# kije/HSLU_I.BA_RAYTRACING.F2501_raytracer

Measured on AMD Instinct MI355X. Metric: Mray/s (primary+secondary, rays counted as the reference casts them), semesterbild@high_resolution, higher is better.
Workload: dtype f32; 1 GPU; semesterbild@high_resolution+anti_aliasing+soft_shadows (text.obj); width=1620, height=1350, rays_per_frame=34992000, rays_traced_per_frame=19683000, pixels_written=1768966, objects=14578, lights=50, parallelism=tiles48x48/1gpu, frames_in_flight=2, build_id=962c7787e075b4de-p0s0w0o6, queue_bytes=0, scene_budget_bytes=2147483648, phases=0

## Files before the change

### hslu_i/ba_raytracing/f2501_raytracer_amd/csrc/rt_api.cpp

```cpp
#include <hip/hip_runtime.h>

#include <algorithm>
#include <chrono>
#include <cmath>
#include <cstdio>
#include <cstdlib>
#include <cstring>
#include <string>
#include <vector>

#include "rt_cell_resolve.h"
#include "rt_host.h"

static void trace_point(hipStream_t stream, const char* what, uint32_t a = 0, uint32_t b = 0, uint32_t c = 0);
#define RC_TRY(expr) do { const int rc_ = (expr); if (rc_ != RT_OK) return rc_; } while (0)

extern "C" {

#ifndef RT_BUILD_ID
#define RT_BUILD_ID "unknown"
#endif
const char* rt_build_id(void) { return RT_BUILD_ID; }

int rt_selftest_exact_math(int device, const float* in, float* out_sqrt, float* out_rcp, uint32_t n) {
  if (!in || !out_sqrt || !out_rcp) return fail(RT_ERR_INVALID_ARG, "null argument");
  if (device < 0 || device >= rt_device_count()) return fail(RT_ERR_INVALID_ARG, "device %d out of range", device);
  HIP_TRY(hipSetDevice(device));
  DevBuf b;
  int rc = b.ensure((size_t)n * 12 + 12);
  if (rc != RT_OK) return rc;
  float* d = (float*)b.p;
  HIP_TRY(hipMemcpy(d, in, (size_t)n * 4, hipMemcpyHostToDevice));
  hipError_t e = (hipError_t)rt_launch_selftest_math(d, d + n, d + 2 * (size_t)n, n, nullptr);
  if (e != hipSuccess) {
    b.release();
    return fail(RT_ERR_HIP, "selftest launch failed: %s", hipGetErrorString(e));
  }
  hipError_t e1 = hipMemcpy(out_sqrt, d + n, (size_t)n * 4, hipMemcpyDeviceToHost);
  hipError_t e2 = hipMemcpy(out_rcp, d + 2 * (size_t)n, (size_t)n * 4, hipMemcpyDeviceToHost);
  b.release();
  if (e1 != hipSuccess || e2 != hipSuccess) return fail(RT_ERR_HIP, "selftest copy failed");
  return RT_OK;
}

// ... 220 lines not shown
    s->cloud_ball_f[0] = p->fw, s->cloud_ball_f[1] = p->fh, s->cloud_ball_f[2] = p->fd;
    rt_scale_cloud(s->cloud_host.data(), n, s->cloud_ball_f, &s->cloud_scaled, s->cloud_ball);
    HIP_TRY(hipMemcpyAsync(s->cloud.p, s->cloud_scaled.data(), n / 3 * 16, hipMemcpyHostToDevice, up.stream));
  }
  P->cloud_sets = (const float4*)s->cloud.p;
  memcpy(P->cloud_centre, s->cloud_ball, 12);
  P->cloud_delta = s->cloud_ball[3];
  rt_beam_constants(p->eps_distance, P);
  const uint32_t cap = p->tuning.shadow_candidate_cap;
  P->cand_cap = cap == RT_CAND_CAP_NONE ? 0u : (cap ? cap : 64u);
  return RT_OK;
}

static int prepare_receiver_flags(rt_scene* s, const rt_params* p, TableUpload& up, RtDevParams* P) {
  hipStream_t stream = up.stream;
  P->recv_flags = nullptr;
  if (p->tuning.no_receiver_flags || P->cand_cap == 0u) s->notes |= RT_NOTE_RECV_FLAGS_OFF_TUNING;
  if (!s->n_cells || !(P->cloud_delta > 0.0f)) s->notes |= RT_NOTE_RECV_FLAGS_OFF_SCENE;
  if (s->dev.n_lights > 8u) s->notes |= RT_NOTE_RECV_FLAGS_OFF_LIGHTS;
  if (p->traversal != RT_TRAVERSAL_BVH) s->notes |= RT_NOTE_RECV_FLAGS_OFF_TRAVERSAL;
  if (p->flags & RT_FLAG_BACKFACE_CULLING) s->notes |= RT_NOTE_RECV_FLAGS_OFF_CULLING;
  if (!p->tuning.no_receiver_flags && P->cand_cap != 0u && s->n_cells && s->dev.n_lights <= 8u && p->traversal == RT_TRAVERSAL_BVH &&
      !(p->flags & RT_FLAG_BACKFACE_CULLING) && P->cloud_delta > 0.0f) {
    const float key[8] = {P->beam_delta, p->eps_distance, P->cloud_centre[0], P->cloud_centre[1], P->cloud_centre[2], 1.f, 0.f, 0.f};
    if (memcmp(key, s->flags_key, sizeof(key)) != 0) {
      RC_TRY(up.begin());
      RtDevParams B = *P;
      B.flag_out = (uint16_t*)s->flags.p;
      B.flag_geo = (const float4*)s->flag_geo.p;
      B.n_cells = s->n_cells;
      B.n_tri_cells = s->n_tri_cells;
      s->cell_lists_built = false;
      s->cell_wide_built = false;
      B.cell_list_out = nullptr;
      const size_t list_bytes = (size_t)s->n_cells * s->dev.n_lights * 16u;
      size_t free_b = 0, total_b = 0;
      const size_t flag_bytes = s->flags.cap + s->flag_geo.cap;
      if (s->dev.n_slots <= 65533u && flag_bytes + list_bytes <= s->budget && hipMemGetInfo(&free_b, &total_b) == hipSuccess &&
          list_bytes <= (free_b + s->cell_lists.cap) / 4 && s->cell_lists.ensure(list_bytes + 64) == RT_OK) {
        HIP_TRY(hipMemsetAsync(s->cell_lists.p, 0xFF, list_bytes, stream));
        B.cell_list_out = (uint16_t*)s->cell_lists.p;
        s->cell_lists_built = true;
      }
      if (!s->cell_lists_built) s->cell_lists.release();
      hipError_t e = (hipError_t)rt_launch_flags(s->dev, B, stream);
      if (e != hipSuccess) return fail(RT_ERR_HIP, "rt_flags_kernel launch failed: %s", hipGetErrorString(e));
      trace_point(stream, "rt_flags_kernel: cells, lights, lists", s->n_cells, s->dev.n_lights, s->cell_lists_built ? 1u : 0u);
      static const char* const prune_env = getenv("RT_CELL_PRUNE");
      static const bool prune_off = prune_env && *prune_env == '0';
      if (s->cell_lists_built && !prune_off) {
        RtCellPruneArgs a{};
        a.flag_geo = (const float*)s->flag_geo.p;
        a.lists = (uint16_t*)s->cell_lists.p;
        a.flags = (uint16_t*)s->flags.p;
        a.n_cells = s->n_cells, a.n_tri_cells = s->n_tri_cells;
        memcpy(a.cloud_centre, P->cloud_centre, 12);
        a.beam_delta = P->beam_delta, a.beam_eps_o = P->beam_eps_o;
        a.mode = RT_PRUNE_FULL;
        e = (hipError_t)rt_launch_cell_prune(s->dev, a, stream);
        if (e != hipSuccess) return fail(RT_ERR_HIP, "rt_cell_prune_kernel launch failed: %s", hipGetErrorString(e));
        trace_point(stream, "rt_cell_prune_kernel: cells, lights", s->n_cells, s->dev.n_lights, 0u);
        static const char* const resolve_env = getenv("RT_CELL_RESOLVE");
        static const bool resolve_off = resolve_env && *resolve_env == '0';
        RtCellResolveArgs r{};
        const size_t temp_bytes = resolve_off ? 0 : rt_cell_resolve_temp_bytes(s->n_cells, s->budget - flag_bytes - list_bytes, &r.chunk_cells);
        if (temp_bytes && s->resolve_work.ensure(temp_bytes) == RT_OK) {
          r.cell = a;
          r.eps_push = P->beam_eps_push, r.eps_ulp = P->beam_eps_ulp;
          r.work = (uint32_t*)s->resolve_work.p;
          static const char* const wide_env = getenv("RT_CELL_WIDE");
          static const bool wide_off = wide_env && *wide_env == '0';
          const size_t used = flag_bytes + list_bytes + temp_bytes;
          const size_t wide_bytes = wide_off || used >= s->budget ? 0 : rt_cell_wide_pool_bytes(s->n_cells, s->dev.n_lights, s->budget - used, &r.wide_cap);
          if (wide_bytes && hipMemGetInfo(&free_b, &total_b) == hipSuccess && wide_bytes <= (free_b + s->cell_wide.cap) / 4 &&
              s->cell_wide.ensure(wide_bytes) == RT_OK) {
            r.wide = (uint16_t*)s->cell_wide.p;
            r.wide_count = (uint32_t*)((char*)s->cell_wide.p + (size_t)r.wide_cap * 2u * RT_CELL_WIDE_SLOTS);
            s->cell_wide_built = true;
          } else {
            r.wide_cap = 0u;
          }
          e = (hipError_t)rt_launch_cell_resolve(s->dev, r, stream);
          if (e != hipSuccess) return fail(RT_ERR_HIP, "rt_cell_resolve_kernel launch failed: %s", hipGetErrorString(e));
          trace_point(stream, "rt_cell_resolve_kernel: cells, lights, cells per chunk", s->n_cells, s->dev.n_lights, r.chunk_cells);
        } else {
          s->resolve_work.release();
        }
      }
      if (!s->cell_lists_built) s->resolve_work.release();
      if (!s->cell_wide_built) s->cell_wide.release();
      memcpy(s->flags_key, key, sizeof(key));
    }
    P->recv_flags = (const uint16_t*)s->flags.p;
    if (s->cell_lists_built && !p->tuning.no_cell_lists) P->cell_lists = (const uint4*)s->cell_lists.p;
    if (P->cell_lists && s->cell_wide_built) P->cell_wide = (const uint32_t*)s->cell_wide.p;
  }
  if (!P->cell_lists) s->notes |= RT_NOTE_CELL_LISTS_OFF;
  return RT_OK;
}

static void copy_frame_shape(rt_scene* s, const rt_params* p, uint32_t* argb_dev, const rt_aux* aux_dev, RtDevParams* P) {
  P->max_depth_reflection = p->max_depth_reflection;
  P->max_depth_refraction = p->max_depth_refraction;
  s->sort_bits_wanted = p->tuning.sort_bits;
  s->lanes_wanted = p->tuning.sub_frames;
  s->phases_wanted = p->tuning.phases;
  s->levels_wanted = p->tuning.levels;
  if (p->win_w) {
    P->win_x0 = p->win_x0, P->win_y0 = p->win_y0, P->win_w = p->win_w, P->win_h = p->win_h;
  } else {
    P->win_x0 = P->win_y0 = 0;
    P->win_w = p->width;
    P->win_h = p->height;
  }
  P->tile_size = p->tile_size ? p->tile_size : 48u;
  P->n_ranks = p->n_ranks;
  P->rank = p->rank;
  P->traversal = p->traversal;
  P->argb = argb_dev;
  if (aux_dev) {
    P->aux_rgb = aux_dev->rgb;
    P->aux_hit_id = aux_dev->hit_id;
    P->aux_hit_t = aux_dev->hit_t;
  }
}

static int take_frame_slot(rt_scene* s, const rt_params* p, hipStream_t stream, RtDevParams* P) {
  int blk = -1, oldest = 0, same = -1;
// ... 767 lines not shown
```

### hslu_i/ba_raytracing/f2501_raytracer_amd/csrc/rt_host.h

```cpp
#pragma once

#include <hip/hip_runtime.h>

#include <string>
#include <vector>

#include "rt_closest.h"
#include "rt_multihit.h"
#include "rt_ray_key.h"
#include "rt_scene_pack.h"

#define fail rt_fail

#define HIP_TRY(expr)                                                                          \
  do {                                                                                         \
    hipError_t e_ = (expr);                                                                    \
    if (e_ != hipSuccess)                                                                      \
      return fail(e_ == hipErrorOutOfMemory ? RT_ERR_OOM : RT_ERR_HIP, "%s failed: %s", #expr, \
                  hipGetErrorString(e_));                                                      \
  } while (0)

#define RT_SLOTS 4
#define RT_LANES 2
#define RT_MAX_DEPTH 64u
// ... 221 lines not shown
  std::vector<uint32_t> sup_host;
  uint32_t sup_key[8] = {0, 0, 0, 0, 0, 0, 0, 0};
  DevBuf costmap;
  std::vector<uint32_t> cost_host;
  uint32_t cost_key[13] = {0, 0, 0, 0, 0, 0, 0, 0, 0, 0, 0, 0, 0};
  bool cost_valid = false, cost_wanted = false;
  uint32_t q_cap = 0, hard_cap = 0, batch_items = 0;
  StreamKey stream_key{};
  uint32_t key_gen = 0;
  uint32_t sticky_notes = 0;
  bool stream_verified = false;
  uint32_t est[RT_LANES][RT_CNT_STRIDE] = {{0}};
  bool est_valid = false;
  uint32_t sort_bits_wanted = 0;
  uint32_t lanes_wanted = 0;
  uint32_t phases_wanted = 0;
  uint32_t levels_wanted = 0;
  uint32_t calm_frames = 1u << 30;
  uint32_t tables_version = 0;
  float aabb_lo[3] = {0.f, 0.f, 0.f}, aabb_hi[3] = {1.f, 1.f, 1.f};
  std::vector<float> aa_host, cloud_host, cloud_scaled;
  std::vector<uint32_t> aa_table;
  uint32_t aa_unique = 0;
  bool aa_dedup = true;
  hipEvent_t tables_ev = nullptr;
  hipStream_t tables_stream = nullptr, last_stream = nullptr;
  bool tables_pending = false, rendered = false;
  float cloud_ball[4] = {0.f, 0.f, 0.f, -1.f};
  DevBuf flag_geo, flags;
  DevBuf cell_lists;
  DevBuf resolve_work;
  DevBuf cell_wide;
  bool cell_wide_built = false;
  bool cell_lists_built = false;
  uint32_t n_cells = 0, n_tri_cells = 0;
  float flags_key[8] = {-1.f, 0.f, 0.f, 0.f, 0.f, 0.f, 0.f, 0.f};
  float cloud_ball_f[3] = {0.f, 0.f, 0.f};
  hipEvent_t frame_ev[RT_SLOTS] = {};
  bool frame_pending[RT_SLOTS] = {};
  uint32_t frame_seq[RT_SLOTS] = {};
  hipStream_t frame_stream[RT_SLOTS] = {};
  uint32_t frame_no = 0;
  int cur_block = 0, last_block = 0;
  int cur_ws = 0;
  int ws_last_block[RT_SLOTS] = {0, 1, 2, 3};
  uint32_t notes = 0;
  size_t queue_bytes = 0;
  RtRefitPlan plan;
  DevBuf plan_dev, upd_dev;
  size_t plan_off[5] = {0, 0, 0, 0, 0};
  void* upd_stage = nullptr;
  size_t upd_stage_cap = 0;
  float* upd_back = nullptr;
  uint64_t sah_created[2] = {0, 0};
  float sah_tri_cost = 2.0f;
  DevBuf sah_dev;
  uint32_t max_leaf = 4;
};


int rt_scene_upload_plan(rt_scene* s, const RtPackedScene& pk);
void rt_scene_release_update(rt_scene* s);

int rt_scene_wait_frames(rt_scene* s);

struct RtRebuildIn {
// ... 30 lines not shown
```

### hslu_i/ba_raytracing/f2501_raytracer_amd/csrc/rt_kernels.hip

```cpp
#include <hip/hip_runtime.h>

#include <stdlib.h>

#include <type_traits>

#include "rt_internal.h"

#define RT_EPS 1.1920929e-7f

#define RT_OPAQUE(v) asm volatile("" : "+v"(v))
#define RT_OPAQUE_S(v) asm volatile("" : "+s"(v))
typedef const __attribute__((address_space(4))) char* rt_kernarg_ptr;
__device__ __forceinline__ rt_kernarg_ptr kernarg_fresh() {
  rt_kernarg_ptr p = (rt_kernarg_ptr)__builtin_amdgcn_kernarg_segment_ptr();
  asm volatile("" : "+s"(p));
  return p;
}
#define RT_KERNARG_OFF_P ((sizeof(RtDevScene) + alignof(RtDevParams) - 1) / alignof(RtDevParams) * alignof(RtDevParams))
static_assert(RT_KERNARG_OFF_P == 88, "RtDevParams follows RtDevScene at kernarg offset 88");
__device__ __forceinline__ const RtDevScene& kernarg_scene() { return *(const RtDevScene*)(const char*)kernarg_fresh(); }
__device__ __forceinline__ const RtDevParams& kernarg_params() {
  return *(const RtDevParams*)((const char*)kernarg_fresh() + RT_KERNARG_OFF_P);
}
#define wave_ballot(pred) __builtin_amdgcn_ballot_w64((bool)(pred))
// ... 447 lines not shown
      if (CULL) h &= wave_ballot(dot(d, n) < 0.75f);
      S.occ |= h;
      return;
    }
    const OccConst k = occluder_constants(m);
    M.row = row;
    M.k.ar = uniform_u(k.ar), M.k.ag = uniform_u(k.ag), M.k.ab = uniform_u(k.ab), M.k.x = uniform_u(k.x);
    M.k.eta2_out = uniform_f(k.eta2_out), M.k.eta2_in = uniform_f(k.eta2_in), M.k.f0x = uniform_f(k.f0x);
    WSTAT(n_miss++);
  }
  WSTAT(n_exec++);
  shadow_add(S, M.k, n, d, h);
}

template <bool CULL>
__device__ __forceinline__ lanemask shadow_accumulate_lane(Shadow& S, const Mat& m, V3 n, V3 d, lanemask h) {
  if (CULL) h &= wave_ballot(m.transmissive || dot(d, n) < 0.75f);
  S.occ |= h & wave_ballot(!m.transmissive);
  const float io = m.transmissive ? m.opacity * (1.0f - fresnel_reflectance_air_red(m, n, -d)) : 0.0f;
  const bool on = lane_of(h);
  const uint32_t di = (uint32_t)__float2uint_rn(clampf(1.0f - io, 0.0f, 1.0f) * RT_SH_SCALE);
  const uint32_t nd = min(S.dec + di, RT_SH_ONE);
  S.dec = on ? nd : S.dec;
  const V3 ab = absorption(m);
  S.fr = on ? S.fr + (uint32_t)__float2uint_rn(ab.x * RT_FILT_SCALE) : S.fr;
  S.fg = on ? S.fg + (uint32_t)__float2uint_rn(ab.y * RT_FILT_SCALE) : S.fg;
  S.fb = on ? S.fb + (uint32_t)__float2uint_rn(ab.z * RT_FILT_SCALE) : S.fb;
  return h;
}

struct WaveCtx {
  uint32_t n_nodes, n_tris, s_nodes, s_tris, s_passes, n_exact, s_exact;
  uint32_t o_exec, o_miss;
#if RT_PROFILE
  unsigned long long t_mark;
  unsigned long long prof[7];
#endif
};

enum { CFG_TABLES_RUNTIME = -1, CFG_TABLES_FLAGS = 1, CFG_TABLES_LISTS = 2 };
struct CfgGeneric {
  static constexpr uint32_t N = 0u;
  static constexpr bool BVH = false;
  static constexpr int TABLES = CFG_TABLES_RUNTIME;
  static constexpr bool POW2_SETS = false;
  static constexpr bool FEW_SPHERES = false;
  static constexpr bool FAR_ORIGINS = false;
  static constexpr bool OCC_MEMO = false;
  static constexpr bool WIDE = false;
};
template <uint32_t N_, int TABLES_>
struct CfgSoft {
  static constexpr uint32_t N = N_;
  static constexpr bool BVH = true;
  static constexpr int TABLES = TABLES_;
  static constexpr bool POW2_SETS = true;
  static constexpr bool FEW_SPHERES = true;
  static constexpr bool FAR_ORIGINS = false;
  static constexpr bool OCC_MEMO = TABLES_ == CFG_TABLES_LISTS;
  static constexpr bool WIDE = TABLES_ == CFG_TABLES_LISTS;
};
struct CfgRays : CfgGeneric {
  static constexpr bool FAR_ORIGINS = true;
};

template <bool CULL, class C = CfgGeneric>
__device__ __forceinline__ Hit nearest_hit(const RtDevScene& sc, const RtDevParams& P, WaveCtx& W,
                                           bool alive, V3 o, V3 d) {
  Hit best;
  best.t = INFINITY;
  best.id = -1;
  const lanemask grp = wave_ballot(alive);
  uint32_t pre = 0xFFFFFFFFu;
  if (sc.n_spheres > 2u && grp) {
    const uint32_t ns = C::FEW_SPHERES ? sc.n_spheres : (sc.n_spheres < 32u ? sc.n_spheres : 32u);
    const int fl = __ffsll((long long)grp) - 1;
    auto first = [&](float v) { return __uint_as_float((uint32_t)__builtin_amdgcn_readlane((int)__float_as_uint(v), fl)); };
    const V3 o0 = mk(first(o.x), first(o.y), first(o.z)), d0 = mk(first(d.x), first(d.y), first(d.z));
    const V3 eo = o - o0, ed = d - d0;
    float so = alive ? fabsf(eo.x) + fabsf(eo.y) + fabsf(eo.z) : 0.0f, sd = alive ? fabsf(ed.x) + fabsf(ed.y) + fabsf(ed.z) : 0.0f;
#pragma unroll
    for (int k = 32; k >= 1; k >>= 1) {
      so = fmaxf(so, __shfl_xor(so, k, 64));
      sd = fmaxf(sd, __shfl_xor(sd, k, 64));
    }
    const uint32_t lane = threadIdx.x & 63u, si = lane < ns ? lane : ns - 1u;
    const float4 sp = vload<float4>(sc, sc.off_spheres + si * 16u);
    const float rad = vload<float>(sc, sc.off_sphere_rad + si * 4u);
    const V3 w = mk(sp.x, sp.y, sp.z) - o0;
    const float tc = fmaxf(dot(w, d0), 0.0f);
    const V3 q = w - d0 * tc;
    const float reach = rad + so + (mag(w) + so + rad) * sd * 1.0001f + 1e-6f;
    pre = (uint32_t)(wave_ballot(dot(q, q) <= reach * reach * 1.0002f) & ((1ull << ns) - 1ull));
// ... 372 lines not shown
          }
          for (uint32_t k = 0; k < nn; k++) {
            if (beam_rejects_all(cc + k, b)) continue;
            lane_put(L.reg, L.count, cc + k, lane_id);
            L.count++;
          }
          if ((L.umbra & grp) == grp && !(MODE == COLLECT_FLAGS && P.cell_list_out)) return;
        } else if (second) {
          in1 = true;
        } else {
          in0 = true;
        }
      }
      if (in0 && in1) {
        lane_put(stk, sp, first1 ? nd.c0 : nd.c1, lane_id);
        sp++;
        next = first1 ? nd.c1 : nd.c0;
      } else if (in0) {
        next = nd.c0;
      } else if (in1) {
        next = nd.c1;
      }
      if (next == RT_NODE_EMPTY) {
        if (sp == 0) break;
        sp--;
        next = (uint32_t)__builtin_amdgcn_readlane((int)stk, (int)sp);
      }
      node = next;
    }
  };
  if (MODE == COLLECT_OWN && have_pre) {
    for (uint32_t i = 0; i < pre_count; i++) {
      const uint32_t slot = (uint32_t)__builtin_amdgcn_readlane((int)pre_reg, (int)i);
      if (beam_rejects_all(slot, grp)) continue;
      if (L.count >= cand_cap) {
        L.count = RT_CAND_OVERFLOW;
        return L;
      }
      lane_put(L.reg, L.count, slot, lane_id);
      L.count++;
      if ((L.umbra & grp) == grp) return L;
    }
    return L;
  }
  if (octant_uniform)
    walk(std::true_type{});
  else
    walk(std::false_type{});
  if (MODE == COLLECT_FLAGS) {
    L.count = (uint32_t)flags_near;
    L.spheres = (uint32_t)(flags_near >> 32);
  }
  return L;
}

template <bool CULL, bool LIST, class C = CfgGeneric>
__device__ __forceinline__ Shadow shadow_ray(const RtDevScene& sc, const RtDevParams& P, WaveCtx& W,
                                             lanemask grp, V3 o, V3 d_raw, float tmax, const CandList& cand, OccMemo& memo) {
  Shadow S;
  shadow_init(S);
  auto count_occluder = [&](const Mat& m, uint32_t row) {
    if (m.transmissive) {
      WSTAT(W.o_exec++);
      WSTAT(W.o_miss += row != memo.row ? 1u : 0u);
      WSTAT(memo.row = row);
    }
  };
// ... 5 lines not shown
#endif
  const unsigned long long t_sph = PROF_T();
  auto test_sphere = [&](uint32_t i) {
    float4 s = sload<float4>(sc, sc.off_spheres + i * 16u);
    float t = 0.0f;
    lanemask h = grp & ~S.occ & wave_ballot(sphere_hit(s, o, d, t));
    h &= wave_ballot(t <= tmax);
    if (h) {
      V3 p = fma_s(d, t, o);
      V3 n = CULL ? normalize(p - mk(s.x, s.y, s.z)) : fast_normalize(p - mk(s.x, s.y, s.z));
      if (C::OCC_MEMO) {
        shadow_accumulate_memo<CULL>(sc, S, memo, sload<uint32_t>(sc, sc.off_sphere_mat + i * 4u), n, d, h, W.o_exec, W.o_miss);
      } else {
        Mat m = load_mat_u(sc, sload<uint32_t>(sc, sc.off_sphere_mat + i * 4u));
        if (CULL && !m.transmissive) h &= wave_ballot(dot(d, n) < 0.75f);
        WSTAT(count_occluder(m, sload<uint32_t>(sc, sc.off_sphere_mat + i * 4u)));
        shadow_accumulate(S, m, n, d, h);
      }
    }
  };
  for (uint32_t bits = cand.spheres & ((!C::FEW_SPHERES && sc.n_spheres >= 32u) ? 0xFFFFFFFFu : ((1u << sc.n_spheres) - 1u)); bits; bits &= bits - 1u)
    test_sphere((uint32_t)__builtin_ctz(bits));
  if constexpr (!C::FEW_SPHERES)
    for (uint32_t i = 32u; i < sc.n_spheres; i++) test_sphere(i);
  if (!LIST && !C::BVH && sc.n_triangles == 0) return S;
#if RT_PROFILE
  RT_OPAQUE(S.dec);
#endif
  PROF_ADD(W, 3, t_sph);
  const unsigned long long t_tri = PROF_T();
  (void)t_tri;

  auto test_tri = [&](uint32_t slot, lanemask lanes) {
    float4 q0 = sload<float4>(sc, sc.off_tri_isect + slot * 48u);
    float4 q1 = sload<float4>(sc, sc.off_tri_isect + slot * 48u + 16u);
    float4 q2 = sload<float4>(sc, sc.off_tri_isect + slot * 48u + 32u);
    float t;
    lanemask h = tri_hit(q0, q1, q2, o, d, lanes & ~S.occ, tmax, t, W.s_exact);
    h &= wave_ballot(t <= tmax);
    if (h) {
      float4 sh = sload<float4>(sc, sc.off_tri_shade + slot * 16u);
      if (C::OCC_MEMO) {
        shadow_accumulate_memo<CULL>(sc, S, memo, __float_as_uint(sh.w), mk(sh.x, sh.y, sh.z), d, h, W.o_exec, W.o_miss);
      } else {
        Mat m = load_mat_u(sc, __float_as_uint(sh.w));
        V3 n = mk(sh.x, sh.y, sh.z);
        if (CULL && !m.transmissive) h &= wave_ballot(dot(d, n) < 0.75f);
        WSTAT(count_occluder(m, __float_as_uint(sh.w)));
        shadow_accumulate(S, m, n, d, h);
      }
    }
  };

  if (!LIST && !C::BVH && P.traversal == RT_TRAVERSAL_LINEAR) {
    for (uint32_t s = 0; s < sc.n_slots; s++)
      if (!(sload<uint32_t>(sc, sc.off_tri_id + s * 4u) & RT_TRI_DUPLICATE)) test_tri(s, grp);
    return S;
  }
  WSTAT(W.s_passes++);

  if (LIST) {
    WSTAT(W.s_tris += cand.count);
    for (uint32_t c = 0; c < cand.count; c++) {
      if (!(grp & ~S.occ)) break;
      uint32_t slot = (uint32_t)__builtin_amdgcn_readlane((int)cand.reg, (int)c);
      test_tri(slot, grp);
    }
#if RT_PROFILE
    RT_OPAQUE(S.dec);
#endif
    PROF_ADD(W, 4, t_tri);
    return S;
  }

  const BoxRay br = box_ray(o, d);
  const float tl = t_limit_slack(tmax);
// ... 104 lines not shown
  const float cint = diff * lI * sig;
  T.mLc = mmc_lc;
  float opac = 1.0f;
  if (FILTERED) {
    const V3 f = shadow_filter(S);
    T.mLc = mk(mmc_lc.x * __builtin_amdgcn_rcpf(f.x), mmc_lc.y * __builtin_amdgcn_rcpf(f.y), mmc_lc.z * __builtin_amdgcn_rcpf(f.z));
    opac = shadow_opacity(S);
  }
  float specf = 0.0f;
  if (has_spec) {
    const V3 rv = fma_s(n, -2.0f * diff, ld);
    const float base = fmaxf(dot(rv, view) * __builtin_amdgcn_rsqf(dot(rv, rv)), 0.0f);
    specf = RT_FAST_TRANS ? fast_pow01(base, fmaxf(mshin * 512.0f, 1.0f)) : powf(base, fmaxf(mshin * 512.0f, 1.0f));
  }
  T.lf = FILTERED ? diff * cint * opac : diff * cint;
  T.sf = FILTERED ? cint * opac * specf : cint * specf;
  T.lit = FILTERED ? __uint_as_float(__float_as_uint(diff) & ((S.dec >> 28) - 1u)) > 0.0f : diff > 0.0f;
  return T;
}

enum { KIND_PRIMARY = 0, KIND_REFL = 1, KIND_REFR = 2 };

#define RT_ACC_SCALE 68719476736.0f
#define RT_ACC_INV_SCALE (1.0f / 68719476736.0f)

struct Wave {
  WaveCtx ctx;
  uint32_t cnt_kind[3], cnt_shadow, cnt_pass, cnt_lanes, cnt_traced;
};

__device__ __forceinline__ void wave_init(Wave& w) {
  w.ctx.n_nodes = w.ctx.n_tris = w.ctx.s_nodes = w.ctx.s_tris = w.ctx.s_passes = w.ctx.n_exact = w.ctx.s_exact = 0;
  w.ctx.o_exec = w.ctx.o_miss = 0;
  w.cnt_kind[0] = w.cnt_kind[1] = w.cnt_kind[2] = 0;
  w.cnt_shadow = w.cnt_pass = w.cnt_lanes = w.cnt_traced = 0;
#if RT_PROFILE
  for (int i = 0; i < 7; i++) w.ctx.prof[i] = 0;
  w.ctx.t_mark = 0;
#endif
}

#define RT_N_COUNTERS 15u
__device__ __forceinline__ void wave_flush_init(const RtDevParams& P, unsigned long long* lds_cnt) {
  if (!P.counters) return;
  if (threadIdx.x < 16u) lds_cnt[threadIdx.x] = 0ull;
  __syncthreads();
}
__device__ __forceinline__ void wave_flush(const Wave& w, const RtDevParams& P, unsigned long long written,
                                           unsigned long long* lds_cnt) {
  if (!P.counters) return;
  uint32_t before = 0u;
  if ((threadIdx.x & 63u) == 0) {
#if RT_PROFILE
    const unsigned long long v[RT_N_COUNTERS] = {w.cnt_kind[0], w.cnt_kind[1], w.cnt_kind[2], w.cnt_shadow, written,
                                                 w.cnt_pass,    w.ctx.prof[6], w.ctx.prof[0],  w.ctx.prof[1], w.ctx.prof[2],
                                                 w.ctx.prof[3], w.ctx.s_passes, w.ctx.prof[4], w.ctx.prof[5], w.cnt_traced};
#elif RT_WORK_STATS == 2
    const unsigned long long v[RT_N_COUNTERS] = {w.cnt_kind[0], w.cnt_kind[1], w.cnt_kind[2], w.cnt_shadow, written,
                                                 w.cnt_pass,    w.cnt_lanes,   w.ctx.o_exec,   w.ctx.o_miss, w.ctx.s_nodes,
                                                 w.ctx.s_tris,  w.ctx.s_passes, w.ctx.n_exact, w.ctx.s_exact, w.cnt_traced};
#else
    const unsigned long long v[RT_N_COUNTERS] = {w.cnt_kind[0], w.cnt_kind[1], w.cnt_kind[2], w.cnt_shadow, written,
                                                 w.cnt_pass,    w.cnt_lanes,   w.ctx.n_nodes,  w.ctx.n_tris, w.ctx.s_nodes,
                                                 w.ctx.s_tris,  w.ctx.s_passes, w.ctx.n_exact, w.ctx.s_exact, w.cnt_traced};
#endif
#pragma unroll
    for (unsigned i = 0; i < RT_N_COUNTERS; i++)
      if (v[i]) atomicAdd(&lds_cnt[i], v[i]);
    before = (uint32_t)__hip_atomic_fetch_add(&lds_cnt[15], 1ull, __ATOMIC_ACQ_REL, __HIP_MEMORY_SCOPE_WORKGROUP);
  }
  before = __builtin_amdgcn_readfirstlane(before);
  if (before + 1u == (blockDim.x >> 6) && (threadIdx.x & 63u) < RT_N_COUNTERS) {
    const uint32_t i = threadIdx.x & 63u;
    unsigned long long v = lds_cnt[i];
    if (v) atomicAdd(&P.counters[(size_t)(blockIdx.x % RT_COUNTER_REPLICAS) * 16u + i], v);
  }
}

struct RayIn {
  V3 o, d_raw;
  float n_start;
  V3 Wt;
  int depth;
  int kind;
  uint32_t pix;
  uint32_t mult;
};

__device__ __forceinline__ int pack_dkm(int depth, int kind, uint32_t mult) {
  return (int)((mult << 10) | ((uint32_t)(depth + 1) << 2) | (uint32_t)kind);
}
__device__ __forceinline__ void unpack_dkm(int v, int& depth, int& kind, uint32_t& mult) {
  kind = v & 3;
// ... 368 lines not shown
      continue;
    }
    CandList cand = cand_unknown();
#if RT_PROFILE == 4
    uint32_t prof_walked = 0, prof_listed = 0, prof_pre = 0;
#endif
    if ((RT_SKIP & 4) && N > 1) {
      cand.count = 0;
      cand.spheres = 0;
    } else if (N > 1 && (C::BVH || P.cloud_delta > 0.0f) && (C::BVH || P.traversal == RT_TRAVERSAL_BVH) && (C::BVH || sc.n_triangles)) {
      V3 centre = mk(L0.x + P.cloud_centre[0], L0.y + P.cloud_centre[1], L0.z + P.cloud_centre[2]);
      const unsigned long long t_c = PROF_T();
      bool walk_tris = true, test_spheres = true;
      if (!CULL && (C::TABLES != CFG_TABLES_RUNTIME || P.recv_flags)) {
        uint32_t tix = threadIdx.x;
        RT_OPAQUE(tix);
        const uint32_t rf = __float_as_uint(stash[10u * 256u + tix]) >> l;
        walk_tris = (use_m & ~wave_ballot(rf & 1u)) != 0ull;
        test_spheres = walk_tris || (use_m & ~wave_ballot((rf >> 8) & 1u)) != 0ull;
      }
      uint32_t pre_reg = 0, pre_count = 0;
      bool have_pre = false;
      if (!CULL && (C::TABLES == CFG_TABLES_LISTS || (C::TABLES == CFG_TABLES_RUNTIME && P.cell_lists)) && walk_tris) {
        uint32_t tix = threadIdx.x;
        RT_OPAQUE(tix);
        const uint32_t cidx = __float_as_uint(stash[RT_STASH_CELL * 256u + tix]);
        uint4 lst = make_uint4(0xFFFFFFFFu, 0xFFFFFFFFu, 0xFFFFFFFFu, 0xFFFFFFFFu);
        if (use && cidx != RT_NO_CELL) lst = P.cell_lists[(size_t)cidx * sc.n_lights + l];
        const lanemask wide_m = C::WIDE ? use_m & wave_ballot(lst.x == RT_CELL_WIDE_HEAD) : 0ull;
        const lanemask unusable = use_m & (wave_ballot(cidx == RT_NO_CELL) | wave_ballot((lst.x & 0xFFFFu) == RT_CELL_LIST_OVERFLOW)) & ~wide_m;
        if (!unusable) {
          have_pre = true;
          const uint32_t lane_id = threadIdx.x & 63u;
          for (lanemask todo = use_m & ~wave_ballot((lst.x & 0xFFFFu) == RT_CELL_LIST_END) & ~wide_m; todo;) {
            const int fl = __ffsll((long long)todo) - 1;
            const uint32_t c = (uint32_t)__builtin_amdgcn_readlane((int)cidx, fl);
            auto add_slot = [&](uint32_t slot) {
              if (slot >= RT_CELL_LIST_OVERFLOW) return;
              const lanemask filled = pre_count >= 64u ? ~0ull : ((1ull << pre_count) - 1ull);
              if (wave_ballot(pre_reg == slot) & filled) return;
              lane_put(pre_reg, pre_count, slot, lane_id);
              pre_count++;
            };
            auto add_pair = [&](uint32_t v) {
              const uint32_t w = (uint32_t)__builtin_amdgcn_readlane((int)v, fl);
              add_slot(w & 0xFFFFu);
              add_slot(w >> 16);
            };
            add_pair(lst.x), add_pair(lst.y), add_pair(lst.z), add_pair(lst.w);
            todo &= ~wave_ballot(cidx == c);
          }
          if constexpr (C::WIDE) {
            if (__builtin_expect(wide_m != 0ull, 0))
            for (lanemask todo = wide_m; todo;) {
              const int fl = __ffsll((long long)todo) - 1;
              const uint32_t c = (uint32_t)__builtin_amdgcn_readlane((int)cidx, fl);
              const uint32_t iw = (uint32_t)__builtin_amdgcn_readlane((int)lst.y, fl);
              const uint4* rec = (const uint4*)(P.cell_wide + (size_t)((iw & 0x7FFFu) | ((iw >> 1) & 0x3FFF8000u)) * RT_CELL_WIDE_DWORDS);
              auto add_slot = [&](uint32_t slot) {
                if (slot >= RT_CELL_LIST_OVERFLOW) return;
                const lanemask filled = pre_count >= 64u ? ~0ull : ((1ull << pre_count) - 1ull);
                if (wave_ballot(pre_reg == slot) & filled) return;
                lane_put(pre_reg, pre_count, slot, lane_id);
                pre_count++;
              };
              auto put_slot = [&](uint32_t slot) {
                if (slot >= RT_CELL_LIST_OVERFLOW) return;
                lane_put(pre_reg, pre_count, slot, lane_id);
                pre_count++;
              };
              const bool fresh = pre_count == 0u;
              for (uint32_t k = 0; k < RT_CELL_WIDE_DWORDS / 4u; k++) {
                const uint4 q = uload(rec + k);
                if (fresh) {
                  put_slot(q.x & 0xFFFFu), put_slot(q.x >> 16), put_slot(q.y & 0xFFFFu), put_slot(q.y >> 16);
                  put_slot(q.z & 0xFFFFu), put_slot(q.z >> 16), put_slot(q.w & 0xFFFFu), put_slot(q.w >> 16);
                } else {
                  add_slot(q.x & 0xFFFFu), add_slot(q.x >> 16), add_slot(q.y & 0xFFFFu), add_slot(q.y >> 16);
                  add_slot(q.z & 0xFFFFu), add_slot(q.z >> 16), add_slot(q.w & 0xFFFFu), add_slot(q.w >> 16);
                }
                if ((q.w >> 16) == RT_CELL_LIST_END) break;
              }
              todo &= ~wave_ballot(cidx == c);
            }
          }
          if (pre_count > 64u) have_pre = false;
        }
      }
#if RT_PROFILE == 4
      prof_walked = (walk_tris && !have_pre) ? 1u : 0u, prof_listed = have_pre ? 1u : 0u, prof_pre = have_pre ? pre_count : 0u;
#endif
#if RT_PROFILE == 6
      if (!CULL && (C::TABLES == CFG_TABLES_LISTS || (C::TABLES == CFG_TABLES_RUNTIME && P.cell_lists)) && walk_tris) {
        uint32_t tix = threadIdx.x;
        RT_OPAQUE(tix);
        const uint32_t cidx = __float_as_uint(stash[RT_STASH_CELL * 256u + tix]);
        uint4 lst = make_uint4(0xFFFFFFFFu, 0xFFFFFFFFu, 0xFFFFFFFFu, 0xFFFFFFFFu);
        if (use && cidx != RT_NO_CELL) lst = P.cell_lists[(size_t)cidx * sc.n_lights + l];
        const bool is_wide = C::WIDE && lst.x == RT_CELL_WIDE_HEAD;
        const lanemask nocell_m = use_m & wave_ballot(cidx == RT_NO_CELL);
        const lanemask plain_m = use_m & wave_ballot((lst.x & 0xFFFFu) == RT_CELL_LIST_OVERFLOW && !is_wide);
        const lanemask wide_m = use_m & wave_ballot(is_wide);
        bool longer = false;
        if (use && is_wide) longer = (P.cell_wide[(size_t)((lst.y & 0x7FFFu) | ((lst.y >> 1) & 0x3FFF8000u)) * RT_CELL_WIDE_DWORDS + 8u] & 0xFFFFu) != RT_CELL_LIST_END;
        W.prof[0] += have_pre ? 0u : 1u;
        W.prof[1] += (!have_pre && nocell_m) ? 1u : 0u;
        W.prof[2] += (!have_pre && !nocell_m && plain_m) ? 1u : 0u;
        W.prof[3] += (!have_pre && !nocell_m && !plain_m) ? 1u : 0u;
        W.prof[4] += (have_pre && wide_m) ? 1u : 0u;
        W.prof[5] += (have_pre && wide_m && !wave_ballot(longer)) ? 1u : 0u;
        W.prof[6] += have_pre ? 1u : 0u;
      }
#endif
      if (test_spheres) {
        cand = collect_light_candidates<CULL, COLLECT_OWN, C>(sc, W, use, sf.p, centre, P, p_first, p_spread, P.cand_cap, nullptr, walk_tris,
                                                              have_pre, pre_reg, pre_count);
      } else {
        cand.count = 0;
        cand.spheres = 0;
      }
#if RT_PROFILE
      RT_OPAQUE(cand.reg);
#endif
      PROF_ADD(W, 1, t_c);
#if RT_SKIP
      if (RT_SKIP & 1) cand.spheres = 0;
      if (RT_SKIP & 2) cand.count = 0;
      if ((RT_SKIP & 8) && cand.count == RT_CAND_OVERFLOW) cand.count = 0, cand.spheres = 0;
#endif
#if RT_PROFILE == 2
      {
        const uint32_t nsph = (uint32_t)__popc(cand.spheres & ((1u << (sc.n_spheres < 32u ? sc.n_spheres : 31u)) - 1u));
        const bool ov = cand.count == RT_CAND_OVERFLOW;
        W.prof[0] += (!ov && cand.count == 0 && nsph == 0) ? 1 : 0;
        W.prof[1] += (!ov && cand.count == 0 && nsph > 0) ? 1 : 0;
        W.prof[2] += (!ov && cand.count >= 1 && cand.count <= 4) ? 1 : 0;
        W.prof[3] += (!ov && cand.count >= 5 && cand.count <= 16) ? 1 : 0;
// ... 1142 lines not shown
```

Measured before the change: 8771 Mray/s.

## Precompute per-cell certain-hit marks for transmissive triangles to skip shadow tests

Adds a precompute kernel that, for each cell and light, marks listed transmissive triangles that every shadow ray from that cell to the light provably passes through, using a conservative geometric rule. The marks are stored ahead of the wide-list pool and signalled through the low bit of the cell_wide pointer. The shadow loop then skips the beam rejection and the triangle intersection test for marked slots and goes straight to accumulating transmission. This saves intersection work per shadow ray, at the cost of an extra one-time kernel, extra memory and a per-lane mark load plus some bookkeeping during candidate-list building. Correctness depends on the conservative rule never marking a triangle that some ray actually misses.

```diff
diff --git a/hslu_i/ba_raytracing/f2501_raytracer_amd/csrc/rt_api.cpp b/hslu_i/ba_raytracing/f2501_raytracer_amd/csrc/rt_api.cpp
--- a/hslu_i/ba_raytracing/f2501_raytracer_amd/csrc/rt_api.cpp
+++ b/hslu_i/ba_raytracing/f2501_raytracer_amd/csrc/rt_api.cpp
@@ -10,6 +10,7 @@
 #include <vector>
 
 #include "rt_cell_resolve.h"
+#include "rt_cell_through.h"
 #include "rt_host.h"
 
 static void trace_point(hipStream_t stream, const char* what, uint32_t a = 0, uint32_t b = 0, uint32_t c = 0);
@@ -296,6 +297,7 @@
       B.n_tri_cells = s->n_tri_cells;
       s->cell_lists_built = false;
       s->cell_wide_built = false;
+      s->cell_marks_bytes = 0;
       B.cell_list_out = nullptr;
       const size_t list_bytes = (size_t)s->n_cells * s->dev.n_lights * 16u;
       size_t free_b = 0, total_b = 0;
@@ -312,8 +314,12 @@
       trace_point(stream, "rt_flags_kernel: cells, lights, lists", s->n_cells, s->dev.n_lights, s->cell_lists_built ? 1u : 0u);
       static const char* const prune_env = getenv("RT_CELL_PRUNE");
       static const bool prune_off = prune_env && *prune_env == '0';
-      if (s->cell_lists_built && !prune_off) {
-        RtCellPruneArgs a{};
+      static const char* const through_env = getenv("RT_CELL_THROUGH");
+      static const bool through_off = through_env && *through_env == '0';
+      size_t mark_bytes = s->cell_lists_built && !through_off ? rt_cell_through_bytes(s->n_cells, s->dev.n_lights, s->budget - flag_bytes - list_bytes) : 0;
+      if (mark_bytes && !(hipMemGetInfo(&free_b, &total_b) == hipSuccess && mark_bytes <= (free_b + s->cell_wide.cap) / 4)) mark_bytes = 0;
+      RtCellPruneArgs a{};
+      if (s->cell_lists_built) {
         a.flag_geo = (const float*)s->flag_geo.p;
         a.lists = (uint16_t*)s->cell_lists.p;
         a.flags = (uint16_t*)s->flags.p;
@@ -321,25 +327,27 @@
         memcpy(a.cloud_centre, P->cloud_centre, 12);
         a.beam_delta = P->beam_delta, a.beam_eps_o = P->beam_eps_o;
         a.mode = RT_PRUNE_FULL;
+      }
+      if (s->cell_lists_built && !prune_off) {
         e = (hipError_t)rt_launch_cell_prune(s->dev, a, stream);
         if (e != hipSuccess) return fail(RT_ERR_HIP, "rt_cell_prune_kernel launch failed: %s", hipGetErrorString(e));
         trace_point(stream, "rt_cell_prune_kernel: cells, lights", s->n_cells, s->dev.n_lights, 0u);
         static const char* const resolve_env = getenv("RT_CELL_RESOLVE");
         static const bool resolve_off = resolve_env && *resolve_env == '0';
         RtCellResolveArgs r{};
-        const size_t temp_bytes = resolve_off ? 0 : rt_cell_resolve_temp_bytes(s->n_cells, s->budget - flag_bytes - list_bytes, &r.chunk_cells);
+        const size_t temp_bytes = resolve_off ? 0 : rt_cell_resolve_temp_bytes(s->n_cells, s->budget - flag_bytes - list_bytes - mark_bytes, &r.chunk_cells);
         if (temp_bytes && s->resolve_work.ensure(temp_bytes) == RT_OK) {
           r.cell = a;
           r.eps_push = P->beam_eps_push, r.eps_ulp = P->beam_eps_ulp;
           r.work = (uint32_t*)s->resolve_work.p;
           static const char* const wide_env = getenv("RT_CELL_WIDE");
           static const bool wide_off = wide_env && *wide_env == '0';
-          const size_t used = flag_bytes + list_bytes + temp_bytes;
+          const size_t used = flag_bytes + list_bytes + temp_bytes + mark_bytes;
           const size_t wide_bytes = wide_off || used >= s->budget ? 0 : rt_cell_wide_pool_bytes(s->n_cells, s->dev.n_lights, s->budget - used, &r.wide_cap);
-          if (wide_bytes && hipMemGetInfo(&free_b, &total_b) == hipSuccess && wide_bytes <= (free_b + s->cell_wide.cap) / 4 &&
-              s->cell_wide.ensure(wide_bytes) == RT_OK) {
-            r.wide = (uint16_t*)s->cell_wide.p;
-            r.wide_count = (uint32_t*)((char*)s->cell_wide.p + (size_t)r.wide_cap * 2u * RT_CELL_WIDE_SLOTS);
+          if (wide_bytes && hipMemGetInfo(&free_b, &total_b) == hipSuccess && mark_bytes + wide_bytes <= (free_b + s->cell_wide.cap) / 4 &&
+              s->cell_wide.ensure(mark_bytes + wide_bytes) == RT_OK) {
+            r.wide = (uint16_t*)((char*)s->cell_wide.p + mark_bytes);
+            r.wide_count = (uint32_t*)((char*)r.wide + (size_t)r.wide_cap * 2u * RT_CELL_WIDE_SLOTS);
             s->cell_wide_built = true;
           } else {
             r.wide_cap = 0u;
@@ -351,13 +359,24 @@
           s->resolve_work.release();
         }
       }
+      if (mark_bytes && (s->cell_wide_built || s->cell_wide.ensure(mark_bytes + 64u) == RT_OK)) {
+        RtCellThroughArgs t{};
+        t.cell = a;
+        t.marks_end = (uint8_t*)s->cell_wide.p + mark_bytes;
+        e = (hipError_t)rt_launch_cell_through(s->dev, t, stream);
+        if (e != hipSuccess) return fail(RT_ERR_HIP, "rt_cell_through_kernel launch failed: %s", hipGetErrorString(e));
+        trace_point(stream, "rt_cell_through_kernel: cells, lights", s->n_cells, s->dev.n_lights, 0u);
+        s->cell_wide_built = true;
+        s->cell_marks_bytes = mark_bytes;
+      }
       if (!s->cell_lists_built) s->resolve_work.release();
       if (!s->cell_wide_built) s->cell_wide.release();
       memcpy(s->flags_key, key, sizeof(key));
     }
     P->recv_flags = (const uint16_t*)s->flags.p;
     if (s->cell_lists_built && !p->tuning.no_cell_lists) P->cell_lists = (const uint4*)s->cell_lists.p;
-    if (P->cell_lists && s->cell_wide_built) P->cell_wide = (const uint32_t*)s->cell_wide.p;
+    if (P->cell_lists && s->cell_wide_built)
+      P->cell_wide = (const uint32_t*)((uintptr_t)((char*)s->cell_wide.p + s->cell_marks_bytes) | (s->cell_marks_bytes ? 1u : 0u));
   }
   if (!P->cell_lists) s->notes |= RT_NOTE_CELL_LISTS_OFF;
   return RT_OK;
diff --git a/hslu_i/ba_raytracing/f2501_raytracer_amd/csrc/rt_cell_through.cpp b/hslu_i/ba_raytracing/f2501_raytracer_amd/csrc/rt_cell_through.cpp
--- /dev/null
+++ b/hslu_i/ba_raytracing/f2501_raytracer_amd/csrc/rt_cell_through.cpp
@@ -0,0 +1,19 @@
+#include <hip/hip_runtime_api.h>
+
+#include "rt_cell_through.h"
+#include "rt_scene_pack.h"
+
+void rt_cell_through_packed(const RtPackedScene& pk, RtCellThroughArgs a) {
+  if (pk.dev.n_lights == 0u || pk.dev.n_lights > 8u || pk.flag_geo.empty() || !a.marks_end) return;
+  a.cell.flag_geo = pk.flag_geo.data();
+  a.cell.n_cells = a.cell.n_cells < pk.n_cells ? a.cell.n_cells : pk.n_cells;
+  a.cell.n_tri_cells = pk.n_tri_cells;
+  const char* base = (const char*)pk.blob.data();
+  for (uint32_t c = 0; c < a.cell.n_cells; c++)
+    rt_cell_through_cell(pk.dev, base, a, c, a.cell.lists + (size_t)c * pk.dev.n_lights * RT_PRUNE_LIST_SLOTS);
+}
+
+size_t rt_cell_through_bytes(uint32_t n_cells, uint32_t n_lights, size_t budget_left) {
+  const size_t n = ((size_t)n_cells * n_lights + 63u) & ~(size_t)63u;
+  return n != 0u && n <= budget_left ? n : 0u;
+}
diff --git a/hslu_i/ba_raytracing/f2501_raytracer_amd/csrc/rt_cell_through.h b/hslu_i/ba_raytracing/f2501_raytracer_amd/csrc/rt_cell_through.h
--- /dev/null
+++ b/hslu_i/ba_raytracing/f2501_raytracer_amd/csrc/rt_cell_through.h
@@ -0,0 +1,99 @@
+#pragma once
+
+#include "rt_cell_resolve.h"
+
+#define RT_THROUGH_NO_RHO_WC 1u
+#define RT_THROUGH_NO_NEAR 2u
+
+#define RT_THROUGH_EPS 1.1920929e-7f
+
+struct RtCellThroughArgs {
+  RtCellPruneArgs cell;
+  uint8_t* marks_end;
+  uint32_t mode;
+};
+
+RT_HD static inline bool rt_through_rule(const RtPruneBeam& B, const float* q, uint32_t mode) {
+  const float v1[3] = {q[0], q[1], q[2]}, c1[3] = {-q[3], -q[4], -q[5]}, c2[3] = {-q[6], -q[7], -q[8]}, X[3] = {q[9], q[10], q[11]};
+  float b[3], bc[3];
+  rt_prune_sub(v1, B.p, b);
+  rt_prune_sub(v1, B.c, bc);
+  const float dr = rt_fadd(B.delta, B.rho);
+  const float nX = rt_prune_norm(X), nb = rt_prune_norm(b), nbc = rt_prune_norm(bc);
+  const float nbo = rt_fadd(nb, B.rho);
+  const float det0 = rt_prune_dot(B.dseg, X);
+  const float ad = fabsf(det0);
+  const float dslack = rt_fadd(rt_fmul(dr, nX), rt_fmul(RT_PRUNE_G, rt_fmul(B.lenp, nX)));
+  if (!(ad > rt_fmul(dslack, 1.001f))) return false;
+  const float sg = det0 < 0.0f ? -1.0f : 1.0f;
+  const float det_hi = rt_fmul(rt_fadd(ad, dslack), 1.00001f);
+  const float det_lo = rt_fmul(rt_fadd(ad, -dslack), 0.99999f);
+  if (!(rt_fdiv(det_lo, B.lenp) > rt_fmul(1.01f, RT_THROUGH_EPS))) return false;
+  const float n2 = rt_prune_norm(c2);
+  float w[3], wc[3];
+  rt_prune_cross(b, c2, w);
+  rt_prune_cross(bc, c2, wc);
+  const float u0 = rt_fmul(rt_prune_dot(B.dseg, w), sg);
+  const float rho_wc = (mode & RT_THROUGH_NO_RHO_WC) ? 0.0f : rt_fmul(B.rho, rt_prune_cross_norm(wc, nbc, n2, true));
+  const float su = rt_fmul(rt_fadd(rt_fadd(rt_fadd(rt_fmul(B.delta, rt_prune_cross_norm(w, nb, n2, true)), rho_wc), rt_fmul(rt_fmul(dr, B.rho), n2)),
+                                   rt_fmul(RT_PRUNE_G, rt_fmul(B.lenp, rt_fmul(n2, nbo)))), 1.00001f);
+  if (!(rt_fadd(u0, -su) > 0.0f)) return false;
+  const float n1 = rt_prune_norm(c1);
+  rt_prune_cross(c1, b, w);
+  rt_prune_cross(c1, bc, wc);
+  const float v0 = rt_fmul(rt_prune_dot(B.dseg, w), sg);
+  const float rho_wc1 = (mode & RT_THROUGH_NO_RHO_WC) ? 0.0f : rt_fmul(B.rho, rt_prune_cross_norm(wc, nbc, n1, true));
+  const float sv = rt_fmul(rt_fadd(rt_fadd(rt_fadd(rt_fmul(B.delta, rt_prune_cross_norm(w, nb, n1, true)), rho_wc1), rt_fmul(rt_fmul(dr, B.rho), n1)),
+                                   rt_fmul(RT_PRUNE_G, rt_fmul(B.lenp, rt_fmul(n1, nbo)))), 1.00001f);
+  if (!(rt_fadd(v0, -sv) > 0.0f)) return false;
+  if (!(rt_fadd(rt_fadd(u0, v0), rt_fmul(rt_fadd(su, sv), 1.00001f)) < det_lo)) return false;
+  const float xb = rt_fmul(rt_prune_dot(X, b), sg);
+  const float tslack = rt_fmul(rt_fadd(rt_fmul(B.rho, nX), rt_fmul(RT_PRUNE_G, rt_fmul(nX, nbo))), 1.00001f);
+  if (!(mode & RT_THROUGH_NO_NEAR)) {
+    const float t_num = rt_fadd(xb, -tslack);
+    const float dmin = rt_fadd(rt_fadd(rt_fmul(rt_fsqrt(rt_prune_dot(B.dseg, B.dseg)), 0.99999f), -B.delta), -B.rho);
+    if (!(t_num > 0.0f && dmin > 0.0f)) return false;
+    if (!(rt_fmul(rt_fdiv(t_num, det_hi), rt_fmul(dmin, 0.9999f)) > rt_fmul(1.01f, RT_THROUGH_EPS))) return false;
+  }
+  if (!(rt_fadd(xb, tslack) < rt_fmul(det_lo, 0.99999f))) return false;
+  return true;
+}
+
+RT_HD static inline bool rt_cell_through_wanted(const RtDevScene& sc, const char* base, const uint16_t* list) {
+  const uint32_t* tri_id = (const uint32_t*)(base + sc.off_tri_id);
+  for (uint32_t l = 0; l < sc.n_lights && l < 8u; l++) {
+    const uint16_t* w = list + (size_t)l * RT_PRUNE_LIST_SLOTS;
+    if (w[0] >= RT_PRUNE_LIST_OVERFLOW) continue;
+    for (uint32_t k = 0; k < RT_PRUNE_LIST_SLOTS && w[k] < RT_PRUNE_LIST_OVERFLOW; k++)
+      if (w[k] < sc.n_slots && (tri_id[w[k]] & RT_TRI_TRANSMISSIVE)) return true;
+  }
+  return false;
+}
+
+RT_HD static inline void rt_cell_through_cell(const RtDevScene& sc, const char* base, const RtCellThroughArgs& a, uint32_t c, const uint16_t* list) {
+  const uint32_t nl = sc.n_lights < 8u ? sc.n_lights : 8u;
+  uint8_t* out = a.marks_end - 1 - (size_t)c * sc.n_lights;
+  RtResolveCell K;
+  const bool on = rt_cell_through_wanted(sc, base, list) && rt_resolve_cell_setup(sc, base, a.cell, c, K);
+  const uint32_t* tri_id = (const uint32_t*)(base + sc.off_tri_id);
+  const float* isect = (const float*)(base + sc.off_tri_isect);
+  for (uint32_t l = 0; l < nl; l++) {
+    uint32_t m = 0u;
+    const uint16_t* w = list + (size_t)l * RT_PRUNE_LIST_SLOTS;
+    if (on && w[0] < RT_PRUNE_LIST_OVERFLOW) {
+      RtPruneBeam B;
+      rt_resolve_beam(sc, base, a.cell, K, l, B);
+      for (uint32_t k = 0; k < RT_PRUNE_LIST_SLOTS; k++) {
+        const uint32_t slot = w[k];
+        if (slot >= RT_PRUNE_LIST_OVERFLOW) break;
+        if (slot < sc.n_slots && (tri_id[slot] & RT_TRI_TRANSMISSIVE) && rt_through_rule(B, isect + 12u * (size_t)slot, a.mode)) m |= 1u << k;
+      }
+    }
+    out[-(ptrdiff_t)l] = (uint8_t)m;
+  }
+}
+
+struct RtPackedScene;
+void rt_cell_through_packed(const RtPackedScene& pk, RtCellThroughArgs a);
+size_t rt_cell_through_bytes(uint32_t n_cells, uint32_t n_lights, size_t budget_left);
+int rt_launch_cell_through(const RtDevScene& sc, const RtCellThroughArgs& a, void* stream);
diff --git a/hslu_i/ba_raytracing/f2501_raytracer_amd/csrc/rt_cell_through.hip b/hslu_i/ba_raytracing/f2501_raytracer_amd/csrc/rt_cell_through.hip
--- /dev/null
+++ b/hslu_i/ba_raytracing/f2501_raytracer_amd/csrc/rt_cell_through.hip
@@ -0,0 +1,19 @@
+#include <hip/hip_runtime.h>
+
+#include "rt_cell_through.h"
+
+#define RT_CELL_THROUGH_WG 256u
+
+__global__ __launch_bounds__(RT_CELL_THROUGH_WG) void rt_cell_through_kernel(RtDevScene sc, RtCellThroughArgs a) {
+  const uint32_t c = blockIdx.x * RT_CELL_THROUGH_WG + threadIdx.x;
+  if (c >= a.cell.n_cells) return;
+  rt_cell_through_cell(sc, sc.base, a, c, a.cell.lists + (size_t)c * sc.n_lights * RT_PRUNE_LIST_SLOTS);
+}
+
+int rt_launch_cell_through(const RtDevScene& sc, const RtCellThroughArgs& a, void* stream) {
+  if (a.cell.n_cells == 0u || sc.n_lights == 0u || sc.n_lights > 8u) return 0;
+  if (!a.marks_end || !a.cell.lists) return (int)hipErrorInvalidValue;
+  hipLaunchKernelGGL(rt_cell_through_kernel, dim3((a.cell.n_cells + RT_CELL_THROUGH_WG - 1u) / RT_CELL_THROUGH_WG), dim3(RT_CELL_THROUGH_WG), 0,
+                     (hipStream_t)stream, sc, a);
+  return (int)hipGetLastError();
+}
diff --git a/hslu_i/ba_raytracing/f2501_raytracer_amd/csrc/rt_host.h b/hslu_i/ba_raytracing/f2501_raytracer_amd/csrc/rt_host.h
--- a/hslu_i/ba_raytracing/f2501_raytracer_amd/csrc/rt_host.h
+++ b/hslu_i/ba_raytracing/f2501_raytracer_amd/csrc/rt_host.h
@@ -277,6 +277,7 @@
   DevBuf resolve_work;
   DevBuf cell_wide;
   bool cell_wide_built = false;
+  size_t cell_marks_bytes = 0;
   bool cell_lists_built = false;
   uint32_t n_cells = 0, n_tri_cells = 0;
   float flags_key[8] = {-1.f, 0.f, 0.f, 0.f, 0.f, 0.f, 0.f, 0.f};
diff --git a/hslu_i/ba_raytracing/f2501_raytracer_amd/csrc/rt_kernels.hip b/hslu_i/ba_raytracing/f2501_raytracer_amd/csrc/rt_kernels.hip
--- a/hslu_i/ba_raytracing/f2501_raytracer_amd/csrc/rt_kernels.hip
+++ b/hslu_i/ba_raytracing/f2501_raytracer_amd/csrc/rt_kernels.hip
@@ -503,6 +503,9 @@
 struct WaveCtx {
   uint32_t n_nodes, n_tris, s_nodes, s_tris, s_passes, n_exact, s_exact;
   uint32_t o_exec, o_miss;
+#if RT_WORK_STATS == 2
+  uint32_t o_tri, o_thru;
+#endif
 #if RT_PROFILE
   unsigned long long t_mark;
   unsigned long long prof[7];
@@ -519,6 +522,7 @@
   static constexpr bool FAR_ORIGINS = false;
   static constexpr bool OCC_MEMO = false;
   static constexpr bool WIDE = false;
+  static constexpr bool THROUGH = false;
 };
 template <uint32_t N_, int TABLES_>
 struct CfgSoft {
@@ -530,6 +534,7 @@
   static constexpr bool FAR_ORIGINS = false;
   static constexpr bool OCC_MEMO = TABLES_ == CFG_TABLES_LISTS;
   static constexpr bool WIDE = TABLES_ == CFG_TABLES_LISTS;
+  static constexpr bool THROUGH = TABLES_ == CFG_TABLES_LISTS;
 };
 struct CfgRays : CfgGeneric {
   static constexpr bool FAR_ORIGINS = true;
@@ -968,7 +973,8 @@
   if (MODE == COLLECT_OWN && have_pre) {
     for (uint32_t i = 0; i < pre_count; i++) {
       const uint32_t slot = (uint32_t)__builtin_amdgcn_readlane((int)pre_reg, (int)i);
-      if (beam_rejects_all(slot, grp)) continue;
+      const bool certain = C::THROUGH && (slot >> 31) != 0u;
+      if (!certain && beam_rejects_all(slot, grp)) continue;
       if (L.count >= cand_cap) {
         L.count = RT_CAND_OVERFLOW;
         return L;
@@ -1040,6 +1046,30 @@
   (void)t_tri;
 
   auto test_tri = [&](uint32_t slot, lanemask lanes) {
+    if constexpr (C::THROUGH && LIST) {
+      lanemask h = lanes & ~S.occ;
+      const bool certain = (slot >> 31) != 0u;
+      slot &= 0xFFFFu;
+      if (!certain) {
+        float4 q0 = sload<float4>(sc, sc.off_tri_isect + slot * 48u);
+        float4 q1 = sload<float4>(sc, sc.off_tri_isect + slot * 48u + 16u);
+        float4 q2 = sload<float4>(sc, sc.off_tri_isect + slot * 48u + 32u);
+        float t;
+        h = tri_hit(q0, q1, q2, o, d, h, tmax, t, W.s_exact);
+        h &= wave_ballot(t <= tmax);
+      }
+      if (h) {
+        float4 sh = sload<float4>(sc, sc.off_tri_shade + slot * 16u);
+#if RT_WORK_STATS == 2
+        const uint32_t exec0 = W.o_exec;
+#endif
+        shadow_accumulate_memo<CULL>(sc, S, memo, __float_as_uint(sh.w), mk(sh.x, sh.y, sh.z), d, h, W.o_exec, W.o_miss);
+#if RT_WORK_STATS == 2
+        W.o_tri += W.o_exec - exec0, W.o_thru += certain ? W.o_exec - exec0 : 0u;
+#endif
+      }
+      return;
+    }
     float4 q0 = sload<float4>(sc, sc.off_tri_isect + slot * 48u);
     float4 q1 = sload<float4>(sc, sc.off_tri_isect + slot * 48u + 16u);
     float4 q2 = sload<float4>(sc, sc.off_tri_isect + slot * 48u + 32u);
@@ -1049,7 +1079,13 @@
     if (h) {
       float4 sh = sload<float4>(sc, sc.off_tri_shade + slot * 16u);
       if (C::OCC_MEMO) {
+#if RT_WORK_STATS == 2
+        const uint32_t exec0 = W.o_exec;
+#endif
         shadow_accumulate_memo<CULL>(sc, S, memo, __float_as_uint(sh.w), mk(sh.x, sh.y, sh.z), d, h, W.o_exec, W.o_miss);
+#if RT_WORK_STATS == 2
+        W.o_tri += W.o_exec - exec0;
+#endif
       } else {
         Mat m = load_mat_u(sc, __float_as_uint(sh.w));
         V3 n = mk(sh.x, sh.y, sh.z);
@@ -1220,6 +1256,9 @@
 __device__ __forceinline__ void wave_init(Wave& w) {
   w.ctx.n_nodes = w.ctx.n_tris = w.ctx.s_nodes = w.ctx.s_tris = w.ctx.s_passes = w.ctx.n_exact = w.ctx.s_exact = 0;
   w.ctx.o_exec = w.ctx.o_miss = 0;
+#if RT_WORK_STATS == 2
+  w.ctx.o_tri = w.ctx.o_thru = 0;
+#endif
   w.cnt_kind[0] = w.cnt_kind[1] = w.cnt_kind[2] = 0;
   w.cnt_shadow = w.cnt_pass = w.cnt_lanes = w.cnt_traced = 0;
 #if RT_PROFILE
@@ -1246,7 +1285,7 @@
 #elif RT_WORK_STATS == 2
     const unsigned long long v[RT_N_COUNTERS] = {w.cnt_kind[0], w.cnt_kind[1], w.cnt_kind[2], w.cnt_shadow, written,
                                                  w.cnt_pass,    w.cnt_lanes,   w.ctx.o_exec,   w.ctx.o_miss, w.ctx.s_nodes,
-                                                 w.ctx.s_tris,  w.ctx.s_passes, w.ctx.n_exact, w.ctx.s_exact, w.cnt_traced};
+                                                 w.ctx.s_tris,  w.ctx.s_passes, w.ctx.o_tri,   w.ctx.o_thru,  w.cnt_traced};
 #else
     const unsigned long long v[RT_N_COUNTERS] = {w.cnt_kind[0], w.cnt_kind[1], w.cnt_kind[2], w.cnt_shadow, written,
                                                  w.cnt_pass,    w.cnt_lanes,   w.ctx.n_nodes,  w.ctx.n_tris, w.ctx.s_nodes,
@@ -1681,12 +1720,34 @@
         if (!unusable) {
           have_pre = true;
           const uint32_t lane_id = threadIdx.x & 63u;
+          uint32_t mark = 0u, n_marking = 0u;
+          bool marks_on = false;
+          if constexpr (C::THROUGH) {
+            const uintptr_t wp = (uintptr_t)P.cell_wide;
+            marks_on = (wp & 1u) != 0u && !wide_m && !(use_m & wave_ballot((lst.x & 0xFFFFu) == RT_CELL_LIST_END));
+            typedef const uint8_t __attribute__((address_space(1))) * GP;
+            if (marks_on && use) mark = ((GP)((wp & ~(uintptr_t)1u) - 0x100000000ull))[(uint32_t)~(cidx * sc.n_lights + l)];
+          }
           for (lanemask todo = use_m & ~wave_ballot((lst.x & 0xFFFFu) == RT_CELL_LIST_END) & ~wide_m; todo;) {
             const int fl = __ffsll((long long)todo) - 1;
             const uint32_t c = (uint32_t)__builtin_amdgcn_readlane((int)cidx, fl);
+            uint32_t mbits = 0u;
+            if constexpr (C::THROUGH) mbits = (uint32_t)__builtin_amdgcn_readlane((int)mark, fl), n_marking++;
             auto add_slot = [&](uint32_t slot) {
               if (slot >= RT_CELL_LIST_OVERFLOW) return;
               const lanemask filled = pre_count >= 64u ? ~0ull : ((1ull << pre_count) - 1ull);
+              if constexpr (C::THROUGH) {
+                const uint32_t marked = (mbits & 1u) << 16;
+                mbits >>= 1;
+                const lanemask there = wave_ballot((pre_reg & 0xFFFFu) == slot) & filled;
+                if (there) {
+                  pre_reg += lane_of(there) ? marked : 0u;
+                  return;
+                }
+                lane_put(pre_reg, pre_count, slot | marked, lane_id);
+                pre_count++;
+                return;
+              }
               if (wave_ballot(pre_reg == slot) & filled) return;
               lane_put(pre_reg, pre_count, slot, lane_id);
               pre_count++;
@@ -1699,13 +1760,16 @@
             add_pair(lst.x), add_pair(lst.y), add_pair(lst.z), add_pair(lst.w);
             todo &= ~wave_ballot(cidx == c);
           }
+          if constexpr (C::THROUGH) {
+            if (marks_on) pre_reg = (pre_reg & 0xFFFFu) | ((pre_reg >> 16) == n_marking ? 0x80000000u : 0u);
+          }
           if constexpr (C::WIDE) {
             if (__builtin_expect(wide_m != 0ull, 0))
             for (lanemask todo = wide_m; todo;) {
               const int fl = __ffsll((long long)todo) - 1;
               const uint32_t c = (uint32_t)__builtin_amdgcn_readlane((int)cidx, fl);
               const uint32_t iw = (uint32_t)__builtin_amdgcn_readlane((int)lst.y, fl);
-              const uint4* rec = (const uint4*)(P.cell_wide + (size_t)((iw & 0x7FFFu) | ((iw >> 1) & 0x3FFF8000u)) * RT_CELL_WIDE_DWORDS);
+              const uint4* rec = (const uint4*)((const uint32_t*)((uintptr_t)P.cell_wide & ~(uintptr_t)1u) + (size_t)((iw & 0x7FFFu) | ((iw >> 1) & 0x3FFF8000u)) * RT_CELL_WIDE_DWORDS);
               auto add_slot = [&](uint32_t slot) {
                 if (slot >= RT_CELL_LIST_OVERFLOW) return;
                 const lanemask filled = pre_count >= 64u ? ~0ull : ((1ull << pre_count) - 1ull);
@@ -1751,7 +1815,7 @@
         const lanemask plain_m = use_m & wave_ballot((lst.x & 0xFFFFu) == RT_CELL_LIST_OVERFLOW && !is_wide);
         const lanemask wide_m = use_m & wave_ballot(is_wide);
         bool longer = false;
-        if (use && is_wide) longer = (P.cell_wide[(size_t)((lst.y & 0x7FFFu) | ((lst.y >> 1) & 0x3FFF8000u)) * RT_CELL_WIDE_DWORDS + 8u] & 0xFFFFu) != RT_CELL_LIST_END;
+        if (use && is_wide) longer = (((const uint32_t*)((uintptr_t)P.cell_wide & ~(uintptr_t)1u))[(size_t)((lst.y & 0x7FFFu) | ((lst.y >> 1) & 0x3FFF8000u)) * RT_CELL_WIDE_DWORDS + 8u] & 0xFFFFu) != RT_CELL_LIST_END;
         W.prof[0] += have_pre ? 0u : 1u;
         W.prof[1] += (!have_pre && nocell_m) ? 1u : 0u;
         W.prof[2] += (!have_pre && !nocell_m && plain_m) ? 1u : 0u;
```

After: 9278 Mray/s (median of 6 runs). +5.8%, better.
